# alibaba/loongcollector

Hardware: AMD Instinct MI355X
Metric: MB/s parsed (512B lines, 10-field regex) per MI355X + HBM-roofline % (higher is better)
Workload: dtype u8

## Files before the change

loongcollector_amd/csrc/gpu_runtime.hip:

```cpp
#include <hip/hip_runtime.h>

#include <type_traits>

#include <algorithm>
#include <atomic>
#include <cstdlib>
#include <map>
#include <mutex>
#include <cstdio>
#include <chrono>
#include <cstring>
#include <thread>
#include <string>
#include <vector>

#include "device_tables.h"
#include "grok_runtime.hpp"
#include "runtime_internal.hpp"
#include "nfa_kernel.hpp"
#include "nfa_wide_kernel.hpp"
#include "nfa_decide_kernel.hpp"
#include "bt_kernel.hpp"
#include "regex_handle.hpp"
#include "sched_kernel.hpp"
// ... 199 lines not shown

void lcReleaseDeviceTables(lc_regex* re) {
    int cur = 0;
    bool haveCur = hipGetDevice(&cur) == hipSuccess;
    {
        LcLazyTdfa& Z = re->lazy;
        for (int d = 0; d < kLcMaxDevices; ++d)
            if (Z.dBlob[d]) {
                Z.retired.emplace_back(d, Z.dBlob[d]);
                Z.dBlob[d] = nullptr;
            }
        for (const auto& r : Z.retired)
            if (hipSetDevice(r.first) == hipSuccess) (void)hipFree(r.second);
        Z.retired.clear();
    }
    for (int d = 0; d < kLcMaxDevices; ++d) {
        if (re->dTdfaBlob[d] || re->dNfaBlob[d] || re->dTdfaWideBlob[d] || re->dScreenBlob[d] || re->dTdfaL2Blob[d] || re->dBtBlob[d]) {
            if (hipSetDevice(d) == hipSuccess) {
                if (re->dBtBlob[d]) (void)hipFree(re->dBtBlob[d]);
                if (re->dTdfaL2Blob[d]) (void)hipFree(re->dTdfaL2Blob[d]);
                if (re->dScreenBlob[d]) (void)hipFree(re->dScreenBlob[d]);
                if (re->dTdfaBlob[d]) (void)hipFree(re->dTdfaBlob[d]);
                if (re->dTdfaWideBlob[d]) (void)hipFree(re->dTdfaWideBlob[d]);
                if (re->dNfaBlob[d]) (void)hipFree(re->dNfaBlob[d]);
            }
            re->dTdfaBlob[d] = re->dNfaBlob[d] = re->dTdfaWideBlob[d] = re->dScreenBlob[d] = re->dTdfaL2Blob[d] = re->dBtBlob[d] = nullptr;
        }
    }
    if (haveCur) (void)hipSetDevice(cur);
}

struct DoneRequest {
    uint32_t* counter = nullptr;
    uint32_t* flag = nullptr;
    uint32_t seq = 0;
    bool armed = false, consumed = false;
};
static thread_local DoneRequest tlsDone;
static thread_local bool tlsJobTableInPlace = false;

static int lcAllowLds(const void* kern, size_t lds) {
    if (lds <= 64 * 1024) return LC_OK;
    int dev = 0;
    HIP_TRY(hipGetDevice(&dev));
    static thread_local std::map<std::pair<const void*, int>, size_t> set;
    size_t& have = set[{kern, dev}];
    if (lds > have) {
        HIP_TRY(hipFuncSetAttribute(kern, hipFuncAttributeMaxDynamicSharedMemorySize, int(lds)));
        have = lds;
    }
    return LC_OK;
}

template <int BLOCK, bool PAIR, bool COMPACT = false>
static int launchTdfaBlock(const void* dBlob, uint32_t blobBytes, uint32_t regBytes, size_t lds, const uint8_t* d_data,
                           const uint32_t* d_off, const uint32_t* d_len, uint32_t sep, uint32_t minLen, uint32_t n, const uint32_t* d_n, const uint32_t* d_order, const uint32_t* d_resume, uint32_t ngroups,
                           int32_t* d_caps, uint8_t* d_status, hipStream_t stream, uint32_t* longFlag = nullptr, uint32_t seq = 0,
                           uint32_t nregsWord = 0, bool pairOne = false) {
    static const bool noGenOff = [] {
        const char* e = getenv("LC_TDFA_NOGEN");
        return e && e[0] == '0';
    }();
    const bool noGen = !PAIR && !noGenOff && (nregsWord & TD_NREGS_NO_GENERAL) != 0;
    constexpr bool kCanMopUp = BLOCK == 256 && !COMPACT;
    const bool mopUp = kCanMopUp && minLen != 0;
    constexpr int kMopUp = kCanMopUp ? kLabMopUp : 0;
    const void* kern;
    const char* name;
    if constexpr (PAIR) {
        constexpr int kOne = kTdfaNoGeneralPrograms | kLabPairOne | (COMPACT ? kLabDmaStage : 0);
        if (pairOne) {
            kern = mopUp ? reinterpret_cast<const void*>(tdfa_stream_kernel<BLOCK, COMPACT, true, kOne | kMopUp>)
                         : reinterpret_cast<const void*>(tdfa_stream_kernel<BLOCK, COMPACT, true, kOne>);
            name = COMPACT ? "tdfa_stream_kernel<compact,nogeneral,pair1,dma>" : "tdfa_stream_kernel<nogeneral,pair1>";
        } else {
            kern = mopUp ? reinterpret_cast<const void*>(tdfa_stream_kernel<BLOCK, COMPACT, true, kMopUp>)
                         : reinterpret_cast<const void*>(tdfa_stream_kernel<BLOCK, COMPACT, true>);
            name = COMPACT ? "tdfa_stream_kernel<compact,pair>" : "tdfa_stream_kernel<pair>";
        }
    } else if constexpr (COMPACT) {
        kern = noGen ? reinterpret_cast<const void*>(tdfa_stream_kernel<BLOCK, true, false, kTdfaNoGeneralPrograms | kLabDmaStage>)
                     : reinterpret_cast<const void*>(tdfa_stream_kernel<BLOCK, true, false, kLabDmaStage>);
        name = noGen ? "tdfa_stream_kernel<compact,nogeneral,dma>" : "tdfa_stream_kernel<compact,dma>";
    } else {
        if (noGen) kern = mopUp ? reinterpret_cast<const void*>(tdfa_stream_kernel<BLOCK, false, false, kTdfaNoGeneralPrograms | kMopUp>)
                                : reinterpret_cast<const void*>(tdfa_stream_kernel<BLOCK, false, false, kTdfaNoGeneralPrograms>);
        else kern = mopUp ? reinterpret_cast<const void*>(tdfa_stream_kernel<BLOCK, false, false, kMopUp>)
                          : reinterpret_cast<const void*>(tdfa_stream_kernel<BLOCK, false, false>);
        name = noGen ? "tdfa_stream_kernel<nogeneral>" : "tdfa_stream_kernel";
    }
    static const size_t extraLds = [] {
        const char* e = getenv("LC_TDFA_EXTRA_LDS");
        return e ? size_t(atol(e)) : size_t(0);
    }();
    lds += extraLds;
    if (const int rc = lcAllowLds(kern, lds); rc != LC_OK) return rc;
    uint32_t grid = (n + BLOCK - 1) / BLOCK;
    if (mopUp) grid = std::min(grid, 256u);
    noteKernel(name);
    const uint32_t* blobArg = static_cast<const uint32_t*>(dBlob);
    uint32_t* doneCounter = nullptr;
    uint32_t* doneFlag = nullptr;
    uint32_t doneSeq = 0;
    if (tlsDone.armed && minLen == 0 && longFlag == nullptr) {
        doneCounter = tlsDone.counter;
        doneFlag = tlsDone.flag;
        doneSeq = tlsDone.seq;
        tlsDone.consumed = true;
    }
    void* args[] = {&d_data, &d_off, &d_len, &sep, &minLen, &n, &d_n, &d_order, &d_resume, &blobArg, &blobBytes, &regBytes, &ngroups,
                    &d_caps, &d_status, &longFlag, &seq, &doneCounter, &doneFlag, &doneSeq};
    HIP_TRY(hipLaunchKernel(kern, dim3(grid), dim3(BLOCK), args, lds, stream));
    return LC_OK;
}

static bool lcPairOneFormat(const std::vector<uint32_t>& blob) {
    const uint32_t po = blob[TD_OFF_PAIR];
    return po != 0 && po / 4 + TP_FORMAT < blob.size() && blob[po / 4 + TP_FORMAT] == 1;
}

static int launchTdfa(lc_regex* re, int dev, const uint8_t* d_data, const uint32_t* d_off, const uint32_t* d_len,
                      uint32_t sep, uint32_t n, const uint32_t* d_n, const uint32_t* d_order, const uint32_t* d_resume, uint32_t ngroups, int32_t* d_caps,
                      uint8_t* d_status, hipStream_t stream);
static int launchTdfaL2Family(lc_regex* re, const uint32_t* hostBlob, const void* dBlob, bool waveByChoice, int dev, const uint8_t* d_data,
                              const uint32_t* d_off, const uint32_t* d_len, uint32_t sep, uint32_t n, const uint32_t* d_n,
                              const uint32_t* d_order, const uint32_t* d_resume, uint32_t ngroups, int32_t* d_caps, uint8_t* d_status,
                              hipStream_t stream, uint32_t* pendingFlag, uint32_t seq) {
// ... 1597 lines not shown
```

loongcollector_amd/csrc/tdfa_kernel.hpp:

```cpp
#pragma once

#include <hip/hip_runtime.h>

#include <type_traits>

#include "../../include/lc_regex_gpu.h"
#include "device_tables.h"

#ifndef LC_TDFA_MIN_WAVES
#define LC_TDFA_MIN_WAVES 1
#endif

typedef uint32_t u32x4 __attribute__((ext_vector_type(4)));
typedef uint32_t __attribute__((address_space(3))) * LdsWordPtr;
typedef u32x4 __attribute__((address_space(3))) * LdsQuadPtr;
typedef const uint8_t __attribute__((address_space(3))) * LdsBytePtr;
typedef const u32x4 __attribute__((address_space(1))) * GlobalQuadPtr;

template <typename RegT>
using LdsRegPtrT = RegT __attribute__((address_space(3))) *;
constexpr uint32_t kTdfaWideMaxLine = 0xFFFFu;

#ifndef LC_TDFA_STAGE_BYTES
#define LC_TDFA_STAGE_BYTES 64
#endif
constexpr uint32_t kTdfaStageBytes = LC_TDFA_STAGE_BYTES;
constexpr int kTdfaLoads = int(kTdfaStageBytes / 16);
constexpr uint32_t kTdfaRowStride = kTdfaStageBytes + 16;
constexpr uint32_t kTdfaStagePerWave = 64 * kTdfaRowStride;

__device__ __forceinline__ void tdfaWaveLdsSync() {
    __builtin_amdgcn_fence(__ATOMIC_ACQ_REL, "wavefront");
    __builtin_amdgcn_wave_barrier();
}

enum { kLabNoStamp = 1, kLabPreClass = 2, kLabGlobalClass = 4, kLabReplicated = 8, kLabNoOutput = 16, kLabNoLoop = 32, kLabNoGeneral = 64,
       kLabOneStamp = 128 ,
       kLabDmaStage = 256 ,
       kLabWaves5 = 512 ,
       kLabNoDmaWait = 1024 ,
       kLabPairOne = 4096 ,
       kLabMopUp = 8192  };
constexpr int kTdfaNoGeneralPrograms = kLabNoGeneral;

template <typename TdfaReg>
__device__ __forceinline__ uint32_t tdfaRegLane(uint32_t tid) {
    if constexpr (sizeof(TdfaReg) == 2) return (tid & ~63u) | ((tid & 31u) << 1) | ((tid >> 5) & 1u);
    else return tid;
}

template <int BLOCK, typename TdfaReg>
__device__ __forceinline__ void tdfaRunMoveList(uint8_t* smem, uint32_t regsBase, uint32_t list, uint32_t pos,
                                                uint32_t tid) {
    TdfaReg* regs = reinterpret_cast<TdfaReg*>(smem + regsBase);
    const uint32_t* hdr = reinterpret_cast<const uint32_t*>(smem);
    const uint32_t* opsStart = reinterpret_cast<const uint32_t*>(smem + hdr[TD_OFF_OPSSTART]);
    const uint16_t* ops = reinterpret_cast<const uint16_t*>(smem + hdr[TD_OFF_OPS]);
    const uint32_t at = opsStart[list];
    const uint32_t cnt = ops[at];
#pragma unroll 1
    for (uint32_t i = 0; i < cnt; ++i) {
        const uint32_t w = ops[at + 1 + i];
        const uint32_t dst = w & 0xFF, src = w >> 8;
        const TdfaReg val = (src == TD_REG_POS) ? TdfaReg(pos) : regs[src * BLOCK + tdfaRegLane<TdfaReg>(tid)];
        regs[dst * BLOCK + tdfaRegLane<TdfaReg>(tid)] = val;
    }
}

__device__ __forceinline__ uint32_t addLowHalf(uint32_t a, uint32_t t) {
    uint32_t r;
    asm("v_add_u32_sdwa %0, %1, %2 dst_sel:DWORD dst_unused:UNUSED_PAD src0_sel:DWORD src1_sel:WORD_0"
        : "=v"(r)
        : "v"(a), "v"(t));
    return r;
}
__device__ __forceinline__ uint32_t addHighHalf(uint32_t a, uint32_t t) {
    uint32_t r;
    asm("v_add_u32_sdwa %0, %1, %2 dst_sel:DWORD dst_unused:UNUSED_PAD src0_sel:DWORD src1_sel:WORD_1"
        : "=v"(r)
        : "v"(a), "v"(t));
    return r;
}

template <int BLOCK, typename TdfaReg, int LAB = 0>
__device__ __forceinline__ void tdfaReplayChunk(uint8_t* smem, u32x4 q, uint32_t t, uint32_t base, uint32_t L,
                                                uint32_t idCol, uint32_t regsBase, uint32_t tid, uint32_t nBytes) {
    typedef LdsRegPtrT<TdfaReg> LdsRegPtr;
    const LdsBytePtr cmap = reinterpret_cast<LdsBytePtr>(TD_CMAP_OFFSET);
    const uint32_t regAddr0 = regsBase + tdfaRegLane<TdfaReg>(tid) * sizeof(TdfaReg);
#pragma unroll 1
    for (uint32_t j = 0; j < nBytes; ++j) {
        const uint32_t word = (j < 8) ? ((j < 4) ? q.x : q.y) : ((j < 12) ? q.z : q.w);
        const uint32_t b = (word >> ((j & 3) * 8)) & 0xFFu;
        uint32_t col = (base + j < L) ? ((LAB & kLabPreClass) ? b : uint32_t(cmap[b])) : idCol;
        if constexpr ((LAB & kLabReplicated) != 0) col = (col << 4) + ((tid & 15u) << 2);
// ... 8 lines not shown
                                                   uint32_t regBytes) {
    if ((blob[TD_NREGS] >> 16) & 0x1FFFu) {
        uint32_t* regs = reinterpret_cast<uint32_t*>(smem + blobBytes);
        for (uint32_t i = threadIdx.x; i < regBytes / 4; i += BLOCK) regs[i] = 0;
    }
}

template <int BLOCK, typename TdfaReg, int LAB = 0>
__device__ __forceinline__ void tdfaWriteResults(uint8_t* smem, uint32_t tileAddr, uint32_t regsBase, uint32_t state, bool live,
                                                 uint32_t line, uint32_t L, uint32_t from, bool permuted, uint32_t nGroupsOut,
                                                 int32_t* __restrict__ caps, uint8_t* __restrict__ status) {
    const uint32_t* hdr = reinterpret_cast<const uint32_t*>(smem);
    const uint32_t tid = threadIdx.x, lane = tid & 63;
    const uint32_t nSlots = hdr[TD_NSLOTS];
    const uint16_t* finalId = reinterpret_cast<const uint16_t*>(smem + hdr[TD_OFF_FINALID]);
    const uint8_t* finalMap = smem + hdr[TD_OFF_FINALMAP];
    const TdfaReg* regs = reinterpret_cast<const TdfaReg*>(smem + regsBase);
    const uint32_t fid = live ? uint32_t(finalId[state]) : 0xFFFFu;
    const bool matched = live && (state != 0) && (fid != 0xFFFFu);
    const uint32_t nOut = 2 * nGroupsOut;
    const uint32_t rl = tdfaRegLane<TdfaReg>(tid);
    const uint32_t foldOff = ((hdr[TD_NREGS] >> 16) & 0x1FFFu) * 16;
    if (foldOff) {
        const uint32_t* fw = reinterpret_cast<const uint32_t*>(smem + foldOff);
        TdfaReg* rw = reinterpret_cast<TdfaReg*>(smem + regsBase) + tdfaRegLane<TdfaReg>(tid);
        const uint32_t nWords = __builtin_amdgcn_readfirstlane(fw[0]);
        for (uint32_t i0 = 0; i0 < nWords; i0 += 64) {
            const uint32_t fwv = (i0 + lane < nWords) ? fw[1 + i0 + lane] : 0xFFFFFF00u;
            const uint32_t cnt = nWords - i0 < 64 ? nWords - i0 : 64;
            for (uint32_t j0 = 0; j0 < cnt; j0 += 4) {
                uint32_t w[4];
                TdfaReg both[4];
#pragma unroll
                for (int k = 0; k < 4; ++k) {
                    w[k] = uint32_t(__builtin_amdgcn_readlane(int(fwv), int((j0 + k) & 63)));
                    both[k] = rw[(w[k] & 0xFFu) * BLOCK];
                }
#pragma unroll
                for (int k = 0; k < 4; ++k) {
                    if (j0 + k >= cnt) break;
                    if (!__any(both[k] != 0)) continue;
#pragma unroll
                    for (int m = 1; m < 4; ++m) {
                        const uint32_t r = (w[k] >> (8 * m)) & 0xFFu;
                        if (r != 0xFFu) {
                            const TdfaReg own = rw[r * BLOCK];
                            rw[r * BLOCK] = both[k] > own ? both[k] : own;
                        }
                    }
                }
            }
        }
    }
    if constexpr ((LAB & kLabPairOne) != 0) {
        const uint32_t* ph = reinterpret_cast<const uint32_t*>(smem + hdr[TD_OFF_PAIR]);
        const uint32_t dOff = ph[TP_OFF_DERIVE];
        if (dOff) {
            const uint32_t* dw = reinterpret_cast<const uint32_t*>(smem + dOff);
            TdfaReg* rw = reinterpret_cast<TdfaReg*>(smem + regsBase) + tdfaRegLane<TdfaReg>(tid);
            const uint32_t nWords = __builtin_amdgcn_readfirstlane(dw[0]);
            for (uint32_t i = 0; i < nWords; ++i) {
                const uint32_t w = __builtin_amdgcn_readfirstlane(dw[1 + i]);
                rw[(w & 0xFFu) * BLOCK] = TdfaReg(rw[((w >> 8) & 0xFFu) * BLOCK] + TdfaReg(w >> 16));
            }
        }
    }
    auto slotValue = [&](uint32_t s) -> int32_t {
        int32_t val = -1;
        if (matched && s < nSlots) {
            const uint32_t m = finalMap[fid * nSlots + s];
            if (m == TD_REG_POS) val = int32_t(L + from);
            else if (m != TD_REG_NONE) val = int32_t(regs[m * BLOCK + rl] + from);
        }
        return val;
    };
    constexpr uint32_t kTileWords = 1024;
    if (!permuted && nOut != 0 && nOut <= kTileWords && __all(live)) {
        int32_t* tile = reinterpret_cast<int32_t*>(smem + tileAddr);
        uint32_t rowsPerPass = kTileWords / nOut;
        if (rowsPerPass > 64) rowsPerPass = 64;
        if (rowsPerPass > 1) rowsPerPass &= ~1u;
        int32_t* gout = caps + size_t(line - lane) * nOut;
        const uint32_t fid0 = __builtin_amdgcn_readfirstlane(fid);
        const bool sameMap = __all(fid == fid0) && fid0 != 0xFFFFu;
        const int32_t end = int32_t(L + from);
        for (uint32_t p0 = 0; p0 < 64; p0 += rowsPerPass) {
            tdfaWaveLdsSync();
            const bool inPass = lane >= p0 && lane - p0 < rowsPerPass;
            int32_t* row = tile + (inPass ? lane - p0 : 0u) * nOut;
            if (sameMap) {
                const uint8_t* map = finalMap + fid0 * nSlots;
                for (uint32_t s0 = 0; s0 < nOut; s0 += 64) {
                    const uint32_t sl = s0 + lane;
                    const uint32_t mapv = (sl < nSlots && sl < nOut) ? uint32_t(map[sl]) : uint32_t(TD_REG_NONE);
                    const uint32_t cnt = nOut - s0 < 64 ? nOut - s0 : 64;
                    for (uint32_t k0 = 0; k0 < cnt; k0 += 8) {
                        int32_t v[8];
#pragma unroll
                        for (int k = 0; k < 8; ++k) {
                            const uint32_t m = uint32_t(__builtin_amdgcn_readlane(int(mapv), int((k0 + k) & 63)));
                            const uint32_t r = m < TD_REG_NONE ? m : 0u;
                            const int32_t reg = int32_t(regs[r * BLOCK + rl] + from);
                            int32_t val = m == TD_REG_POS ? end : reg;
                            val = m == TD_REG_NONE ? -1 : val;
                            v[k] = state != 0 ? val : -1;
                        }
                        if (inPass) {
#pragma unroll
                            for (int k = 0; k < 8; ++k)
                                if (k0 + k < cnt) row[s0 + k0 + k] = v[k];
                        }
                    }
                }
            } else if (inPass) {
#pragma unroll 4
                for (uint32_t s = 0; s < nOut; ++s) row[s] = slotValue(s);
            }
            tdfaWaveLdsSync();
            const uint32_t rows = 64 - p0 < rowsPerPass ? 64 - p0 : rowsPerPass;
            const uint32_t total = rows * nOut;
            int32_t* g = gout + size_t(p0) * nOut;
            if ((reinterpret_cast<uintptr_t>(g) & 15u) == 0 && (total & 3u) == 0) {
                typedef int32_t i32x4 __attribute__((ext_vector_type(4)));
                const uint32_t nq = total / 4;
                i32x4 q[4];
#pragma unroll
                for (int i = 0; i < 4; ++i) {
                    const uint32_t at = lane + 64u * uint32_t(i);
                    if (at < nq) q[i] = *reinterpret_cast<const i32x4 __attribute__((address_space(3)))*>(tileAddr + at * 16u);
                }
#pragma unroll
                for (int i = 0; i < 4; ++i) {
                    const uint32_t at = lane + 64u * uint32_t(i);
                    if (at < nq) __builtin_nontemporal_store(q[i], reinterpret_cast<i32x4*>(g) + at);
                }
            } else {
                for (uint32_t d = lane; d < total; d += 64) g[d] = tile[d];
            }
        }
    } else if (live) {
        int32_t* out = caps + size_t(line) * nOut;
        for (uint32_t s = 0; s < nOut; ++s) out[s] = slotValue(s);
    }
// ... 21 lines not shown
```

loongcollector_amd/csrc/tdfa_stream_kernel.hpp:

```cpp
#pragma once

#include "tdfa_kernel.hpp"

#ifndef LC_TDFA_STREAM_CHUNK
#define LC_TDFA_STREAM_CHUNK 8
#endif
#ifndef LC_TDFA_GCLASS
#define LC_TDFA_GCLASS 0
#endif
#ifndef LC_TDFA_STAMP_ISA
#define LC_TDFA_STAMP_ISA 1
#endif
#ifndef LC_TDFA_ROW_ALIGN
#define LC_TDFA_ROW_ALIGN 1
#endif
#ifndef LC_TDFA_STREAM_WAVES
#define LC_TDFA_STREAM_WAVES 4
#endif

constexpr uint32_t kTdfaIdColByteAddr = TD_ID_COL * 4;

template <int NB, bool CHECKED, typename TdfaReg, int LAB>
__device__ __forceinline__ uint32_t tdfaStreamChunk(uint32_t t, const uint32_t (&col)[NB], uint32_t (&ncol)[NB],
                                                    const uint32_t (&nwords)[NB / 4], uint32_t nbase, uint32_t L, uint32_t idCol,
// ... 24 lines not shown
#ifndef LC_TDFA_STREAM_NO_SCHED_BARRIER
        __builtin_amdgcn_sched_barrier(0);
#endif
    }
    seenOut = seen | t;
    return t;
}

template <int BLOCK, int NB, bool CHECKED, typename TdfaReg, int LAB = 0>
__device__ __forceinline__ uint32_t tdfaStreamPairChunk(uint32_t t, const uint32_t (&colp)[NB / 2], uint32_t (&na)[NB / 2],
                                                        uint32_t (&nc)[NB / 2], const uint32_t (&nwords)[NB / 4], uint32_t nbase,
                                                        uint32_t L, uint32_t cmapA, uint32_t idAAddr,
                                                        const uint32_t (&ptt)[NB / 2], uint32_t (&tt)[NB / 2], uint32_t pbase,
                                                        uint32_t regAddr0, uint32_t& seenOut) {
    typedef LdsRegPtrT<TdfaReg> LdsRegPtr;
    constexpr uint32_t kRegShift = (BLOCK == 1024 ? 12 : BLOCK == 512 ? 11 : BLOCK == 256 ? 10 : BLOCK == 128 ? 9 : 8) -
                                   (sizeof(TdfaReg) == 2 ? 1 : 0);
    uint32_t seen = 0;
    uint32_t pos = pbase;
#pragma unroll
    for (int p = 0; p < NB / 2; ++p) {
        t = *reinterpret_cast<LdsWordPtr>(addLowHalf(colp[p], t));
        tt[p] = t;
        uint32_t b0, b1;
        asm volatile("v_bfe_u32 %0, %1, %2, 8" : "=v"(b0) : "v"(nwords[p >> 1]), "n"((p & 1) * 16));
        asm volatile("v_bfe_u32 %0, %1, %2, 8" : "=v"(b1) : "v"(nwords[p >> 1]), "n"((p & 1) * 16 + 8));
        if constexpr (CHECKED) {
            na[p] = *reinterpret_cast<LdsHalfPtr>((nbase + 2 * p < L) ? cmapA + b0 * 2 : idAAddr);
            nc[p] = *reinterpret_cast<LdsBytePtr>((nbase + 2 * p + 1 < L) ? TD_CMAP_OFFSET + b1 : kTdfaIdColByteAddr);
        } else {
            na[p] = *reinterpret_cast<LdsHalfPtr>(cmapA + b0 * 2);
            nc[p] = *reinterpret_cast<LdsBytePtr>(TD_CMAP_OFFSET + b1);
        }
        if constexpr ((LAB & kLabOneStamp) != 0) {
            *reinterpret_cast<LdsRegPtr>(regAddr0 + (((ptt[p] >> 16) & 0xFu) << kRegShift)) = TdfaReg(pos);
            asm volatile("v_add_u32 %0, 2, %0" : "+v"(pos));
        } else {
            const uint32_t r0 = (ptt[p] >> 16) & 0xFFu, r1 = ptt[p] >> 24;
            *reinterpret_cast<LdsRegPtr>(regAddr0 + (r0 << kRegShift)) = TdfaReg(pos);
            asm volatile("v_add_u32 %0, 1, %0" : "+v"(pos));
            *reinterpret_cast<LdsRegPtr>(regAddr0 + (r1 << kRegShift)) = TdfaReg(pos);
            asm volatile("v_add_u32 %0, 1, %0" : "+v"(pos));
        }
        if constexpr ((LAB & kLabNoGeneral) == 0)
            if (p > 0) seen |= tt[p - 1];
#ifndef LC_TDFA_STREAM_NO_SCHED_BARRIER
        __builtin_amdgcn_sched_barrier(0);
#endif
    }
    seenOut = seen | t;
    return t;
}

template <int BLOCK, int NB, bool CHECKED, typename TdfaReg>
__device__ __forceinline__ uint32_t tdfaStreamPair1Chunk(uint32_t t, const uint32_t (&colp)[NB / 2], uint32_t (&na)[NB / 2],
                                                         uint32_t (&nc)[NB / 2], const uint32_t (&nwords)[NB / 4], uint32_t nbase,
                                                         uint32_t L, uint32_t cmapA, uint32_t idAAddr,
                                                         const uint32_t (&ptt)[NB / 2], uint32_t (&tt)[NB / 2], uint32_t pbase,
                                                         uint32_t regAddr0, const uint8_t* __restrict__ gcmap8 = nullptr) {
    typedef LdsRegPtrT<TdfaReg> LdsRegPtr;
    constexpr uint32_t kRegShift = (BLOCK == 1024 ? 12 : BLOCK == 512 ? 11 : BLOCK == 256 ? 10 : BLOCK == 128 ? 9 : 8) -
                                   (sizeof(TdfaReg) == 2 ? 1 : 0);
#pragma unroll
    for (int p = 0; p < NB / 2; ++p) {
        t = *reinterpret_cast<LdsWordPtr>(addLowHalf(colp[p], t));
        tt[p] = t;
        uint32_t b0, b1;
        asm volatile("v_bfe_u32 %0, %1, %2, 8" : "=v"(b0) : "v"(nwords[p >> 1]), "n"((p & 1) * 16));
        asm volatile("v_bfe_u32 %0, %1, %2, 8" : "=v"(b1) : "v"(nwords[p >> 1]), "n"((p & 1) * 16 + 8));
        if constexpr (CHECKED) {
            na[p] = *reinterpret_cast<LdsHalfPtr>((nbase + 2 * p < L) ? cmapA + b0 * 2 : idAAddr);
            nc[p] = *reinterpret_cast<LdsBytePtr>((nbase + 2 * p + 1 < L) ? TD_CMAP_OFFSET + b1 : kTdfaIdColByteAddr);
        } else {
            na[p] = *reinterpret_cast<LdsHalfPtr>(cmapA + b0 * 2);
#if LC_TDFA_GCLASS
            nc[p] = gcmap8[b1];
#else
            nc[p] = *reinterpret_cast<LdsBytePtr>(TD_CMAP_OFFSET + b1);
#endif
        }
#if LC_TDFA_STAMP_ISA
        if constexpr (LC_TDFA_ROW_ALIGN == 1) {
            uint32_t ra, delta, addr, val;
            asm("v_bfe_u32 %0, %1, 16, 7" : "=v"(ra) : "v"(ptt[p]));
            asm("v_lshl_add_u32 %0, %1, %2, %3" : "=v"(addr) : "v"(ra), "n"(kRegShift), "v"(regAddr0));
            asm("v_bfe_u32 %0, %1, 23, 1" : "=v"(delta) : "v"(ptt[p]));
            const uint32_t posU = __builtin_amdgcn_readfirstlane(pbase) + uint32_t(2 * p);
            asm("v_add_u32 %0, %1, %2" : "=v"(val) : "s"(posU), "v"(delta));
            *reinterpret_cast<LdsRegPtr>(addr) = TdfaReg(val);
        } else
#endif
        {
            const uint32_t ra = (ptt[p] >> 16) & 0x7Fu;
            *reinterpret_cast<LdsRegPtr>(regAddr0 + (ra << kRegShift)) = TdfaReg(pbase + uint32_t(2 * p) + ((ptt[p] >> 23) & 1u));
        }
#ifndef LC_TDFA_STREAM_NO_SCHED_BARRIER
        __builtin_amdgcn_sched_barrier(0);
#endif
    }
    return t;
}
template <int BLOCK, int NP, typename TdfaReg>
__device__ __forceinline__ void tdfaSettleDoubles(const uint32_t (&ptt)[NP], uint32_t pbase, uint32_t regAddr0) {
    typedef LdsRegPtrT<TdfaReg> LdsRegPtr;
    constexpr uint32_t kRegShift = (BLOCK == 1024 ? 12 : BLOCK == 512 ? 11 : BLOCK == 256 ? 10 : BLOCK == 128 ? 9 : 8) -
                                   (sizeof(TdfaReg) == 2 ? 1 : 0);
    uint32_t any = 0;
#pragma unroll
    for (int p = 0; p < NP; ++p) any |= ptt[p];
    if (!__any(int32_t(any) < 0)) return;
#pragma unroll
    for (int p = 0; p < NP; ++p) {
        if (int32_t(ptt[p]) < 0) {
            const LdsRegPtr reg = reinterpret_cast<LdsRegPtr>(regAddr0 + (((ptt[p] >> 24) & 0x7Fu) << kRegShift));
            const TdfaReg val = TdfaReg(pbase + uint32_t(2 * p) + 1u);
            const TdfaReg cur = *reg;
            *reg = cur > val ? cur : val;
        }
    }
}

__device__ __forceinline__ void tdfaDmaLoad16(uint32_t ldsDst, uint64_t base, uint32_t off) {
    uint32_t keep;
    asm volatile("s_mov_b32 %0, m0\n\ts_mov_b32 m0, %2\n\ts_nop 0\n\tglobal_load_lds_dwordx4 %1, %3\n\ts_mov_b32 m0, %0"
                 : "=&s"(keep)
                 : "v"(off), "s"(ldsDst), "s"(base)
                 : "memory");
}
__device__ __forceinline__ void tdfaDmaWait() { asm volatile("s_waitcnt vmcnt(0)" ::: "memory"); }
__device__ __forceinline__ void tdfaLdsDrain() { asm volatile("s_waitcnt lgkmcnt(0)" ::: "memory"); }

template <int BLOCK, bool COMPACT, bool PAIR, int LAB>
__device__ __forceinline__ void tdfaStreamBody(
    const uint8_t* __restrict__ data, const uint32_t* __restrict__ off, const uint32_t* __restrict__ len, uint32_t sepBytes,
    uint32_t minLen, uint32_t nLines, const uint32_t* __restrict__ nLinesPtr, const uint32_t* __restrict__ order,
    const uint32_t* __restrict__ resume, const uint32_t* __restrict__ blob, uint32_t blobBytes, uint32_t regBytes,
    uint32_t nGroupsOut, int32_t* __restrict__ caps, uint8_t* __restrict__ status, uint32_t* __restrict__ longFlag,
    uint32_t launchSeq, uint32_t blockId) {
    static_assert(kTdfaStageBytes == 64 || kTdfaStageBytes == 128, "4 or 8 16-byte segments per stage");
    constexpr int kLoads = kTdfaLoads;
    static_assert(!PAIR || (LAB & kLabPreClass) == 0, "no pre-classified pairs");
    typedef typename std::conditional<COMPACT, uint16_t, uint32_t>::type TdfaReg;
    typedef LdsRegPtrT<TdfaReg> LdsRegPtr;
    constexpr uint32_t kRowStride = COMPACT ? kTdfaStageBytes : kTdfaRowStride;
    constexpr uint32_t kStagePerWave = 64 * kRowStride;
    constexpr bool DMA = COMPACT && (LAB & kLabDmaStage) != 0 && kTdfaStageBytes == 64;
    constexpr bool PAIR1 = PAIR && (LAB & kLabPairOne) != 0;
    static_assert(!PAIR1 || (LAB & kLabNoGeneral) != 0, "one-stamp pair tables have no general register programs");
    extern __shared__ __attribute__((aligned(16))) uint8_t smem[];
    const uint32_t tid = threadIdx.x;
    if (nLinesPtr) {
        const uint32_t dyn = *nLinesPtr;
        nLines = dyn < nLines ? dyn : nLines;
    }
    if (minLen && longFlag && __atomic_load_n(longFlag, __ATOMIC_RELAXED) < launchSeq) return;
    if (minLen) {
        const uint32_t s0 = blockId * BLOCK + tid;
        bool mine = false;
        if (s0 < nLines) {
            const uint32_t ln = order ? order[s0] : s0;
            uint32_t l0 = len ? len[ln] : off[ln + 1] - off[ln] - sepBytes;
            if (resume) {
                const uint32_t f0 = resume[ln];
                l0 -= f0 < l0 ? f0 : l0;
            }
            mine = l0 >= minLen;
        }
        volatile uint32_t* flag = reinterpret_cast<volatile uint32_t*>(smem);
        if (tid == 0) *flag = 0;
        __syncthreads();
        if (mine) *flag = 1;
        __syncthreads();
        const bool any = *flag != 0;
        __syncthreads();
        if (!any) return;
    }
    {
        const uint4* src = reinterpret_cast<const uint4*>(blob);
        uint4* dst = reinterpret_cast<uint4*>(smem);
        for (uint32_t i = tid; i < blobBytes / 16; i += BLOCK) dst[i] = src[i];
        tdfaClearRegisters<BLOCK>(smem, blob, blobBytes, regBytes);
        if constexpr (PAIR1) {
            if (((blob[TD_NREGS] >> 16) & 0x1FFFu) == 0) {
                uint32_t* regs = reinterpret_cast<uint32_t*>(smem + blobBytes);
                for (uint32_t i = threadIdx.x; i < regBytes / 4; i += BLOCK) regs[i] = 0;
            }
        }
    }
    __syncthreads();
    const uint32_t* hdr = reinterpret_cast<const uint32_t*>(smem);
    const uint32_t rowBytes = hdr[TD_ROW_BYTES];
    const uint32_t idCol = hdr[TD_ID_COL];
    const uint32_t regsBase = blobBytes;
    const uint32_t dummyT = PAIR1 ? ((hdr[TD_NREGS] & 0xFFFFu) - 1) << 16 : PAIR ? ((hdr[TD_NREGS] & 0xFFFFu) - 1) * 0x01010000u : (((hdr[TD_NREGS] & 0xFFFFu) - 1) * BLOCK * uint32_t(sizeof(TdfaReg))) << 16;
    uint32_t t = hdr[TD_START_ROW];
    TdfaPairInfo pi{};
    uint32_t idAAddr = 0;
    auto walkRow = [&](uint32_t singleRow) {
        return PAIR ? pi.base + ((singleRow & 0xFFFFu) - TD_TRANS_OFFSET) / rowBytes * pi.rowBytes : singleRow;
    };
    if constexpr (PAIR) {
// ... 81 lines not shown
    u32x4 in[kLoads];
    u32x4 W[kLoads];
    if constexpr (DMA) {
        dmaStage(0);
        tdfaDmaWait();
#pragma unroll
        for (int k = 0; k < kLoads; ++k) W[k] = *reinterpret_cast<LdsQuadPtr>(myRow + ((uint32_t(k) * 16) ^ mySwizzle));
    } else {
#pragma unroll
        for (int i = 0; i < kLoads; ++i) {
            in[i] = u32x4{0, 0, 0, 0};
            if (seg < srcSpan[i]) in[i] = *reinterpret_cast<GlobalQuadPtr>(dataAligned + srcOff[i]);
        }
        tdfaWaveLdsSync();
#pragma unroll
        for (int i = 0; i < kLoads; ++i) *reinterpret_cast<LdsQuadPtr>(dstAddr[i]) = in[i];
        tdfaWaveLdsSync();
#pragma unroll
        for (int i = 0; i < kLoads; ++i) {
            in[i] = u32x4{0, 0, 0, 0};
            if (kTdfaStageBytes + seg < srcSpan[i]) in[i] = *reinterpret_cast<GlobalQuadPtr>(dataAligned + (srcOff[i] + kTdfaStageBytes));
        }
#pragma unroll
        for (int k = 0; k < kLoads; ++k) W[k] = *reinterpret_cast<LdsQuadPtr>(myRow + ((uint32_t(k) * 16) ^ mySwizzle));
    }
    constexpr int NB = LC_TDFA_STREAM_CHUNK;
    constexpr int kChunksPerStage = int(kTdfaStageBytes) / NB;
    auto rowWord = [&](int w) -> uint32_t {
        const u32x4& q = W[(w >> 2) & (kLoads - 1)];
        return (w & 3) == 0 ? q.x : (w & 3) == 1 ? q.y : (w & 3) == 2 ? q.z : q.w;
    };
    constexpr int NC = PAIR ? NB / 2 : NB;
    uint32_t col[NC], ptt[NC];
    {
        const uint32_t base0 = 0u - head;
#pragma unroll
        for (int j = 0; j < NB; ++j) {
            const uint32_t b = (rowWord(j >> 2) >> ((j & 3) * 8)) & 0xFFu;
            uint32_t c;
            if constexpr ((LAB & kLabPreClass) != 0) c = (base0 + j < L) ? b : idCol;
            else if (PAIR && (j & 1) == 0) c = *reinterpret_cast<LdsHalfPtr>((base0 + j < L) ? pi.cmapA + b * 2 : idAAddr);
            else c = *reinterpret_cast<LdsBytePtr>((base0 + j < L) ? TD_CMAP_OFFSET + b : kTdfaIdColByteAddr);
            if constexpr (PAIR) {
                if ((j & 1) == 0) col[j / 2] = c;
                else col[j / 2] += c;
            } else {
                col[j] = c;
            }
        }
#pragma unroll
        for (int j = 0; j < NC; ++j) ptt[j] = dummyT;
    }
    uint32_t pbase = 0;

    if constexpr ((LAB & kLabNoLoop) != 0) maxStages = 0;
    for (uint32_t s = 0; s < maxStages; ++s) {
        if constexpr (DMA) {
            tdfaLdsDrain();
            dmaStage((s + 1) * kTdfaStageBytes);
        } else {
            tdfaWaveLdsSync();
#pragma unroll
            for (int i = 0; i < kLoads; ++i) *reinterpret_cast<LdsQuadPtr>(dstAddr[i]) = in[i];
            tdfaWaveLdsSync();
            const uint32_t nextOff = (s + 2) * kTdfaStageBytes;
#pragma unroll
            for (int i = 0; i < kLoads; ++i) {
                in[i] = u32x4{0, 0, 0, 0};
                if (nextOff + seg < srcSpan[i]) in[i] = *reinterpret_cast<GlobalQuadPtr>(dataAligned + (srcOff[i] + nextOff));
            }
        }
        auto runChunks = [&](auto allFullTag, auto c0Tag, auto c1Tag) -> bool {
        constexpr bool ALLFULL = decltype(allFullTag)::value;
        constexpr int C0 = decltype(c0Tag)::value, C1 = decltype(c1Tag)::value;
#pragma unroll
        for (int c = C0; c < C1; ++c) {
            const uint32_t base = s * kTdfaStageBytes + uint32_t(c) * NB - head;
            if constexpr (!ALLFULL && PAIR1) {
                if (c > 0 && __all(s * kTdfaStageBytes + uint32_t(c) * NB >= head + L)) return true;
            }
            const uint32_t nbase = base + NB;
            const bool waveFull = PAIR1 && waveMaxHead <= s * kTdfaStageBytes + uint32_t(c + 1) * NB &&
                                  waveMinSpan >= s * kTdfaStageBytes + uint32_t(c + 2) * NB;
            const bool fullNext = ALLFULL || waveFull || (nbase < L && L - nbase >= uint32_t(NB));
            const uint32_t entry = t;
            uint32_t nwords[NB / 4], cwords[4] = {0, 0, 0, 0};
#pragma unroll
            for (int w = 0; w < NB / 4; ++w) {
                nwords[w] = rowWord(((c + 1) * NB / 4 + w) & (kLoads * 4 - 1));
                cwords[w] = rowWord(c * NB / 4 + w);
            }
            uint32_t ncol[NC], tt[NC], seen;
            bool general;
            if constexpr (PAIR1) {
                uint32_t na[NC], nc[NC];
                if (ALLFULL || waveFull || __all(fullNext)) t = tdfaStreamPair1Chunk<BLOCK, NB, false, TdfaReg>(t, col, na, nc, nwords, nbase, L, pi.cmapA, idAAddr, ptt, tt, pbase, regAddr0, reinterpret_cast<const uint8_t*>(blob) + TD_CMAP_OFFSET);
                else t = tdfaStreamPair1Chunk<BLOCK, NB, true, TdfaReg>(t, col, na, nc, nwords, nbase, L, pi.cmapA, idAAddr, ptt, tt, pbase, regAddr0);
                tdfaSettleDoubles<BLOCK, NC, TdfaReg>(ptt, pbase, regAddr0);
#pragma unroll
                for (int j = 0; j < NC; ++j) ncol[j] = na[j] + nc[j];
                seen = 0;
                general = false;
            } else if constexpr (PAIR) {
                uint32_t na[NC], nc[NC];
                if (__all(fullNext)) t = tdfaStreamPairChunk<BLOCK, NB, false, TdfaReg, LAB>(t, col, na, nc, nwords, nbase, L, pi.cmapA, idAAddr, ptt, tt, pbase, regAddr0, seen);
                else t = tdfaStreamPairChunk<BLOCK, NB, true, TdfaReg, LAB>(t, col, na, nc, nwords, nbase, L, pi.cmapA, idAAddr, ptt, tt, pbase, regAddr0, seen);
#pragma unroll
                for (int j = 0; j < NC; ++j) ncol[j] = na[j] + nc[j];
                general = (LAB & kLabNoGeneral) ? false : (seen & ((TP_GENERAL << 16) | (TP_GENERAL << 24))) != 0;
            } else {
                if (__all(fullNext)) t = tdfaStreamChunk<NB, false, TdfaReg, LAB>(t, col, ncol, nwords, nbase, L, idCol, ptt, tt, pbase, regAddr0, seen);
                else t = tdfaStreamChunk<NB, true, TdfaReg, LAB>(t, col, ncol, nwords, nbase, L, idCol, ptt, tt, pbase, regAddr0, seen);
                general = (LAB & kLabNoGeneral) ? false : (seen & (TD_OP_GENERAL << 16)) != 0;
            }
            if (__any(general)) {
                const u32x4 q = {cwords[0], cwords[1], cwords[2], cwords[3]};
                uint32_t single = entry;
                if constexpr (PAIR) single = TD_TRANS_OFFSET + ((entry & 0xFFFFu) - pi.base) / pi.rowBytes * rowBytes;
                tdfaReplayChunk<BLOCK, TdfaReg, LAB>(smem, q, single, base, L, idCol, regsBase, tid, NB);
#pragma unroll
                for (int j = 0; j < NC; ++j) tt[j] = dummyT;
            }
            if constexpr (DMA) {
                if (c == kChunksPerStage - 2) {
                    if constexpr ((LAB & kLabNoDmaWait) == 0) tdfaDmaWait();
#pragma unroll
                    for (int k = 0; k < kLoads - 1; ++k) W[k] = *reinterpret_cast<LdsQuadPtr>(myRow + ((uint32_t(k) * 16) ^ mySwizzle));
                } else if (c == kChunksPerStage - 1) {
                    W[kLoads - 1] = *reinterpret_cast<LdsQuadPtr>(myRow + ((uint32_t(kLoads - 1) * 16) ^ mySwizzle));
                }
            } else if ((c + 1) * NB % 16 == 0) {
                const int k = ((c + 1) * NB / 16 - 1) & (kLoads - 1);
                W[k] = *reinterpret_cast<LdsQuadPtr>(myRow + ((uint32_t(k) * 16) ^ mySwizzle));
            }
#pragma unroll
            for (int j = 0; j < NC; ++j) {
                col[j] = ncol[j];
                ptt[j] = tt[j];
            }
            pbase = base;
        }
        return false;
        };
        {
            using std::integral_constant;
            constexpr integral_constant<int, 0> k0{};
            constexpr integral_constant<int, 2> k2{};
            constexpr integral_constant<int, kChunksPerStage - 1> kLast{};
            constexpr integral_constant<int, kChunksPerStage> kEnd{};
            const uint32_t s0 = s * kTdfaStageBytes;
            const bool headsPastChunk0 = PAIR1 && waveMaxHead <= s0 + uint32_t(NB);
            const bool headsPastChunk2 = PAIR1 && waveMaxHead <= s0 + 3u * uint32_t(NB);
            const bool allNextInside = PAIR1 && waveMinSpan >= s0 + kTdfaStageBytes + uint32_t(NB);
            const bool nextInsideButLast = PAIR1 && waveMinSpan >= s0 + kTdfaStageBytes;
            if (headsPastChunk0 && allNextInside) {
                (void)runChunks(std::true_type{}, k0, kEnd);
            } else if (kChunksPerStage == 8 && headsPastChunk2 && allNextInside) {
                if (!runChunks(std::false_type{}, k0, k2)) (void)runChunks(std::true_type{}, k2, kEnd);
            } else if (kChunksPerStage == 8 && headsPastChunk0 && nextInsideButLast) {
                (void)runChunks(std::true_type{}, k0, kLast);
                (void)runChunks(std::false_type{}, kLast, kEnd);
            } else {
                (void)runChunks(std::false_type{}, k0, kEnd);
            }
        }
        if (__all((t & 0xFFFFu) == deadRow || s + 1 >= myStages)) break;
    }
    if constexpr (DMA) tdfaDmaWait();
    if constexpr (PAIR1) {
        constexpr uint32_t kRegShift = (BLOCK == 1024 ? 12 : BLOCK == 512 ? 11 : BLOCK == 256 ? 10 : BLOCK == 128 ? 9 : 8) -
                                       (sizeof(TdfaReg) == 2 ? 1 : 0);
#pragma unroll
        for (int j = 0; j < NC; ++j)
            *reinterpret_cast<LdsRegPtr>(regAddr0 + (((ptt[j] >> 16) & 0x7Fu) << kRegShift)) = TdfaReg(pbase + 2 * j + ((ptt[j] >> 23) & 1u));
        tdfaSettleDoubles<BLOCK, NC, TdfaReg>(ptt, pbase, regAddr0);
    } else if constexpr ((LAB & kLabNoStamp) == 0) {
        if constexpr (PAIR) {
            constexpr uint32_t kRegShift = (BLOCK == 1024 ? 12 : BLOCK == 512 ? 11 : BLOCK == 256 ? 10 : BLOCK == 128 ? 9 : 8) -
                                           (sizeof(TdfaReg) == 2 ? 1 : 0);
#pragma unroll
            for (int j = 0; j < NC; ++j) {
                *reinterpret_cast<LdsRegPtr>(regAddr0 + (((ptt[j] >> 16) & 0xFFu) << kRegShift)) = TdfaReg(pbase + 2 * j);
                *reinterpret_cast<LdsRegPtr>(regAddr0 + ((ptt[j] >> 24) << kRegShift)) = TdfaReg(pbase + 2 * j + 1);
            }
        } else {
#pragma unroll
            for (int j = 0; j < NC; ++j)
                *reinterpret_cast<LdsRegPtr>(addHighHalf(regAddr0, ptt[j])) = TdfaReg(pbase + j);
        }
    }

    if constexpr ((LAB & kLabNoOutput) != 0) {
        if (live && t == 0x12345u) status[line] = 3;
        return;
    }
    const uint32_t state = PAIR ? ((t & 0xFFFFu) - pi.base) / pi.rowBytes : ((t & 0xFFFFu) - TD_TRANS_OFFSET) / rowBytes;
    tdfaWriteResults<BLOCK, TdfaReg, LAB>(smem, stageBase, regsBase, state, live, line, L, from, order != nullptr, nGroupsOut, caps,
                                     status);
    };
    walkBlock(blockId);
}

template <int BLOCK, bool COMPACT, bool PAIR = false, int LAB = 0>
__global__ __launch_bounds__(BLOCK, (LAB & kLabWaves5) ? 5 : LC_TDFA_STREAM_WAVES) void tdfa_stream_kernel(
    const uint8_t* __restrict__ data, const uint32_t* __restrict__ off, const uint32_t* __restrict__ len, uint32_t sepBytes,
    uint32_t minLen, uint32_t nLines, const uint32_t* __restrict__ nLinesPtr, const uint32_t* __restrict__ order,
    const uint32_t* __restrict__ resume, const uint32_t* __restrict__ blob, uint32_t blobBytes, uint32_t regBytes,
    uint32_t nGroupsOut, int32_t* __restrict__ caps, uint8_t* __restrict__ status, uint32_t* __restrict__ longFlag,
    uint32_t launchSeq, uint32_t* __restrict__ doneCounter, uint32_t* __restrict__ doneFlag, uint32_t doneSeq) {
    if constexpr (!COMPACT && (LAB & kLabMopUp) != 0) {
        if (minLen) {
            if (longFlag && __atomic_load_n(longFlag, __ATOMIC_RELAXED) < launchSeq) return;
            const uint32_t nBlocks = (nLines + BLOCK - 1) / BLOCK;
            for (uint32_t b = blockIdx.x; b < nBlocks; b += gridDim.x) {
                tdfaStreamBody<BLOCK, COMPACT, PAIR, LAB>(data, off, len, sepBytes, minLen, nLines, nLinesPtr, order, resume, blob, blobBytes,
                                                         regBytes, nGroupsOut, caps, status, longFlag, launchSeq, b);
                __syncthreads();
            }
            tdfaSignalDone(doneCounter, doneFlag, doneSeq);
            return;
        }
    }
    tdfaStreamBody<BLOCK, COMPACT, PAIR, LAB>(data, off, len, sepBytes, minLen, nLines, nLinesPtr, order, resume, blob, blobBytes,
                                             regBytes, nGroupsOut, caps, status, longFlag, launchSeq, blockIdx.x);
    tdfaSignalDone(doneCounter, doneFlag, doneSeq);
}

struct TdfaJob {
// ... 21 lines not shown
```

Measured before the change: 3.193 million.

## Add deferred tag-register stamps and in-register derive for pair1 TDFA output

Adds a kLabDeferStamps kernel variant that buffers per-lane register-stamp events in two registers and flushes them to LDS only when a wave has a real pending event, instead of writing a stamp for every pair position. Separately, the output path computes derived register values in VGPRs via readlane chains when the row is small and the wave shares one final map, avoiding per-lane LDS derive writes. The deferred variant is gated by an env var defaulting to off, so only the row-in-registers output path is active by default. The trade-off is extra ALU and wave-vote work in the stream loop against fewer LDS stores.

```diff
diff --git a/loongcollector_amd/csrc/gpu_runtime.hip b/loongcollector_amd/csrc/gpu_runtime.hip
--- a/loongcollector_amd/csrc/gpu_runtime.hip
+++ b/loongcollector_amd/csrc/gpu_runtime.hip
@@ -275,6 +275,9 @@
     return LC_OK;
 }
 
+#ifndef LC_TDFA_DEFER_STAMPS_DEFAULT
+#define LC_TDFA_DEFER_STAMPS_DEFAULT 0
+#endif
 template <int BLOCK, bool PAIR, bool COMPACT = false>
 static int launchTdfaBlock(const void* dBlob, uint32_t blobBytes, uint32_t regBytes, size_t lds, const uint8_t* d_data,
                            const uint32_t* d_off, const uint32_t* d_len, uint32_t sep, uint32_t minLen, uint32_t n, const uint32_t* d_n, const uint32_t* d_order, const uint32_t* d_resume, uint32_t ngroups,
@@ -296,6 +299,14 @@
             kern = mopUp ? reinterpret_cast<const void*>(tdfa_stream_kernel<BLOCK, COMPACT, true, kOne | kMopUp>)
                          : reinterpret_cast<const void*>(tdfa_stream_kernel<BLOCK, COMPACT, true, kOne>);
             name = COMPACT ? "tdfa_stream_kernel<compact,nogeneral,pair1,dma>" : "tdfa_stream_kernel<nogeneral,pair1>";
+            if constexpr (COMPACT && LC_TDFA_ROW_ALIGN == 1) {
+                const char* e = getenv("LC_TDFA_DEFER_STAMPS");
+                const bool defer = e ? e[0] != '0' : bool(LC_TDFA_DEFER_STAMPS_DEFAULT);
+                if (defer) {
+                    kern = reinterpret_cast<const void*>(tdfa_stream_kernel<BLOCK, COMPACT, true, kOne | kLabDeferStamps>);
+                    name = "tdfa_stream_kernel<compact,nogeneral,pair1,dma,defer>";
+                }
+            }
         } else {
             kern = mopUp ? reinterpret_cast<const void*>(tdfa_stream_kernel<BLOCK, COMPACT, true, kMopUp>)
                          : reinterpret_cast<const void*>(tdfa_stream_kernel<BLOCK, COMPACT, true>);
diff --git a/loongcollector_amd/csrc/tdfa_kernel.hpp b/loongcollector_amd/csrc/tdfa_kernel.hpp
--- a/loongcollector_amd/csrc/tdfa_kernel.hpp
+++ b/loongcollector_amd/csrc/tdfa_kernel.hpp
@@ -40,7 +40,8 @@
        kLabWaves5 = 512 ,
        kLabNoDmaWait = 1024 ,
        kLabPairOne = 4096 ,
-       kLabMopUp = 8192  };
+       kLabMopUp = 8192 ,
+       kLabDeferStamps = 16384  };
 constexpr int kTdfaNoGeneralPrograms = kLabNoGeneral;
 
 template <typename TdfaReg>
@@ -155,17 +156,27 @@
             }
         }
     }
+    constexpr uint32_t kTileWords = 1024;
+    const bool viaTile = !permuted && nOut != 0 && nOut <= kTileWords && __all(live);
+    const uint32_t fid0 = __builtin_amdgcn_readfirstlane(fid);
+    const bool sameMap = __all(fid == fid0) && fid0 != 0xFFFFu;
+    constexpr uint32_t kRowRegs = 24;
+    uint32_t nDerive = 0;
+    const uint32_t* deriveWords = nullptr;
     if constexpr ((LAB & kLabPairOne) != 0) {
         const uint32_t* ph = reinterpret_cast<const uint32_t*>(smem + hdr[TD_OFF_PAIR]);
         const uint32_t dOff = ph[TP_OFF_DERIVE];
         if (dOff) {
-            const uint32_t* dw = reinterpret_cast<const uint32_t*>(smem + dOff);
-            TdfaReg* rw = reinterpret_cast<TdfaReg*>(smem + regsBase) + tdfaRegLane<TdfaReg>(tid);
-            const uint32_t nWords = __builtin_amdgcn_readfirstlane(dw[0]);
-            for (uint32_t i = 0; i < nWords; ++i) {
-                const uint32_t w = __builtin_amdgcn_readfirstlane(dw[1 + i]);
-                rw[(w & 0xFFu) * BLOCK] = TdfaReg(rw[((w >> 8) & 0xFFu) * BLOCK] + TdfaReg(w >> 16));
-            }
+            deriveWords = reinterpret_cast<const uint32_t*>(smem + dOff) + 1;
+            nDerive = __builtin_amdgcn_readfirstlane(deriveWords[-1]);
+        }
+    }
+    const bool rowInRegs = viaTile && sameMap && nOut <= kRowRegs && nDerive <= 64;
+    if (!rowInRegs && nDerive != 0) {
+        TdfaReg* rw = reinterpret_cast<TdfaReg*>(smem + regsBase) + tdfaRegLane<TdfaReg>(tid);
+        for (uint32_t i = 0; i < nDerive; ++i) {
+            const uint32_t w = __builtin_amdgcn_readfirstlane(deriveWords[i]);
+            rw[(w & 0xFFu) * BLOCK] = TdfaReg(rw[((w >> 8) & 0xFFu) * BLOCK] + TdfaReg(w >> 16));
         }
     }
     auto slotValue = [&](uint32_t s) -> int32_t {
@@ -177,21 +188,56 @@
         }
         return val;
     };
-    constexpr uint32_t kTileWords = 1024;
-    if (!permuted && nOut != 0 && nOut <= kTileWords && __all(live)) {
+    if (viaTile) {
         int32_t* tile = reinterpret_cast<int32_t*>(smem + tileAddr);
         uint32_t rowsPerPass = kTileWords / nOut;
         if (rowsPerPass > 64) rowsPerPass = 64;
         if (rowsPerPass > 1) rowsPerPass &= ~1u;
         int32_t* gout = caps + size_t(line - lane) * nOut;
-        const uint32_t fid0 = __builtin_amdgcn_readfirstlane(fid);
-        const bool sameMap = __all(fid == fid0) && fid0 != 0xFFFFu;
         const int32_t end = int32_t(L + from);
+        int32_t rowv[kRowRegs];
+        if (rowInRegs) {
+            const uint8_t* map = finalMap + fid0 * nSlots;
+            const uint32_t mapv = (lane < nSlots && lane < nOut) ? uint32_t(map[lane]) : uint32_t(TD_REG_NONE);
+            const uint32_t dwv = lane < nDerive ? deriveWords[lane] : 0u;
+            uint32_t root = mapv, dsum = 0;
+            for (uint32_t i = nDerive; i-- > 0;) {
+                const uint32_t w = uint32_t(__builtin_amdgcn_readlane(int(dwv), int(i)));
+                const bool hit = root == (w & 0xFFu);
+                root = hit ? (w >> 8) & 0xFFu : root;
+                dsum += hit ? w >> 16 : 0u;
+            }
+#pragma unroll
+            for (int k = 0; k < int(kRowRegs); k += 2) {
+                if (uint32_t(k) < nOut) {
+#pragma unroll
+                    for (int h = 0; h < 2; ++h) {
+                        const uint32_t m = uint32_t(__builtin_amdgcn_readlane(int(root), k + h));
+                        const uint32_t d = uint32_t(__builtin_amdgcn_readlane(int(dsum), k + h));
+                        const uint32_t r = m < TD_REG_NONE ? m : 0u;
+                        const int32_t reg = int32_t(TdfaReg(regs[r * BLOCK + rl] + TdfaReg(d)) + from);
+                        int32_t val = m == TD_REG_POS ? end : reg;
+                        val = m == TD_REG_NONE ? -1 : val;
+                        rowv[k + h] = state != 0 ? val : -1;
+                    }
+                }
+            }
+        }
         for (uint32_t p0 = 0; p0 < 64; p0 += rowsPerPass) {
             tdfaWaveLdsSync();
             const bool inPass = lane >= p0 && lane - p0 < rowsPerPass;
             int32_t* row = tile + (inPass ? lane - p0 : 0u) * nOut;
-            if (sameMap) {
+            if (rowInRegs) {
+                if (inPass) {
+#pragma unroll
+                    for (int k = 0; k < int(kRowRegs); k += 2) {
+                        if (uint32_t(k) < nOut) {
+                            row[k] = rowv[k];
+                            row[k + 1] = rowv[k + 1];
+                        }
+                    }
+                }
+            } else if (sameMap) {
                 const uint8_t* map = finalMap + fid0 * nSlots;
                 for (uint32_t s0 = 0; s0 < nOut; s0 += 64) {
                     const uint32_t sl = s0 + lane;
diff --git a/loongcollector_amd/csrc/tdfa_stream_kernel.hpp b/loongcollector_amd/csrc/tdfa_stream_kernel.hpp
--- a/loongcollector_amd/csrc/tdfa_stream_kernel.hpp
+++ b/loongcollector_amd/csrc/tdfa_stream_kernel.hpp
@@ -100,12 +100,44 @@
     return t;
 }
 
-template <int BLOCK, int NB, bool CHECKED, typename TdfaReg>
+__device__ __forceinline__ uint32_t tdfaDeferEvent(uint32_t entry, uint32_t posU) {
+    return (entry & 0x00FF0000u) | posU;
+}
+template <int BLOCK, typename TdfaReg>
+__device__ __forceinline__ void tdfaDeferStore(uint32_t ev, uint32_t regAddr0) {
+    typedef LdsRegPtrT<TdfaReg> LdsRegPtr;
+    constexpr uint32_t kRegShift = (BLOCK == 1024 ? 12 : BLOCK == 512 ? 11 : BLOCK == 256 ? 10 : BLOCK == 128 ? 9 : 8) -
+                                   (sizeof(TdfaReg) == 2 ? 1 : 0);
+    uint32_t ra, delta, addr;
+    asm("v_bfe_u32 %0, %1, 16, 7" : "=v"(ra) : "v"(ev));
+    asm("v_lshl_add_u32 %0, %1, %2, %3" : "=v"(addr) : "v"(ra), "n"(kRegShift), "v"(regAddr0));
+    asm("v_bfe_u32 %0, %1, 23, 1" : "=v"(delta) : "v"(ev));
+    *reinterpret_cast<LdsRegPtr>(addr) = TdfaReg(ev + delta);
+}
+template <int BLOCK, typename TdfaReg>
+__device__ __forceinline__ void tdfaDeferFlush(uint32_t& e0, uint32_t& e1, uint32_t dummyEv, uint32_t regAddr0) {
+    tdfaDeferStore<BLOCK, TdfaReg>(e1, regAddr0);
+    tdfaDeferStore<BLOCK, TdfaReg>(e0, regAddr0);
+    e0 = dummyEv;
+    e1 = dummyEv;
+}
+template <int BLOCK, typename TdfaReg>
+__device__ __forceinline__ void tdfaDeferPush(uint32_t entry, uint32_t posU, uint32_t& e0, uint32_t& e1, uint32_t dummyEv,
+                                              uint32_t regAddr0) {
+    const uint32_t ev = tdfaDeferEvent(entry, posU);
+    const bool real = (entry & 0x007F0000u) != dummyEv;
+    e1 = real ? e0 : e1;
+    e0 = real ? ev : e0;
+    if (__any(e1 != dummyEv)) tdfaDeferFlush<BLOCK, TdfaReg>(e0, e1, dummyEv, regAddr0);
+}
+
+template <int BLOCK, int NB, bool CHECKED, typename TdfaReg, int LAB = 0>
 __device__ __forceinline__ uint32_t tdfaStreamPair1Chunk(uint32_t t, const uint32_t (&colp)[NB / 2], uint32_t (&na)[NB / 2],
                                                          uint32_t (&nc)[NB / 2], const uint32_t (&nwords)[NB / 4], uint32_t nbase,
                                                          uint32_t L, uint32_t cmapA, uint32_t idAAddr,
                                                          const uint32_t (&ptt)[NB / 2], uint32_t (&tt)[NB / 2], uint32_t pbase,
-                                                         uint32_t regAddr0, const uint8_t* __restrict__ gcmap8 = nullptr) {
+                                                         uint32_t regAddr0, uint32_t& e0, uint32_t& e1, uint32_t dummyEv,
+                                                         const uint8_t* __restrict__ gcmap8 = nullptr) {
     typedef LdsRegPtrT<TdfaReg> LdsRegPtr;
     constexpr uint32_t kRegShift = (BLOCK == 1024 ? 12 : BLOCK == 512 ? 11 : BLOCK == 256 ? 10 : BLOCK == 128 ? 9 : 8) -
                                    (sizeof(TdfaReg) == 2 ? 1 : 0);
@@ -127,6 +159,10 @@
             nc[p] = *reinterpret_cast<LdsBytePtr>(TD_CMAP_OFFSET + b1);
 #endif
         }
+        if constexpr ((LAB & kLabNoStamp) != 0) {
+        } else if constexpr ((LAB & kLabDeferStamps) != 0) {
+            tdfaDeferPush<BLOCK, TdfaReg>(ptt[p], __builtin_amdgcn_readfirstlane(pbase) + uint32_t(2 * p), e0, e1, dummyEv, regAddr0);
+        } else
 #if LC_TDFA_STAMP_ISA
         if constexpr (LC_TDFA_ROW_ALIGN == 1) {
             uint32_t ra, delta, addr, val;
@@ -148,8 +184,9 @@
     }
     return t;
 }
-template <int BLOCK, int NP, typename TdfaReg>
-__device__ __forceinline__ void tdfaSettleDoubles(const uint32_t (&ptt)[NP], uint32_t pbase, uint32_t regAddr0) {
+template <int BLOCK, int NP, typename TdfaReg, int LAB = 0>
+__device__ __forceinline__ void tdfaSettleDoubles(const uint32_t (&ptt)[NP], uint32_t pbase, uint32_t regAddr0, uint32_t& e0,
+                                                  uint32_t& e1, uint32_t dummyEv) {
     typedef LdsRegPtrT<TdfaReg> LdsRegPtr;
     constexpr uint32_t kRegShift = (BLOCK == 1024 ? 12 : BLOCK == 512 ? 11 : BLOCK == 256 ? 10 : BLOCK == 128 ? 9 : 8) -
                                    (sizeof(TdfaReg) == 2 ? 1 : 0);
@@ -157,6 +194,7 @@
 #pragma unroll
     for (int p = 0; p < NP; ++p) any |= ptt[p];
     if (!__any(int32_t(any) < 0)) return;
+    if constexpr ((LAB & kLabDeferStamps) != 0) tdfaDeferFlush<BLOCK, TdfaReg>(e0, e1, dummyEv, regAddr0);
 #pragma unroll
     for (int p = 0; p < NP; ++p) {
         if (int32_t(ptt[p]) < 0) {
@@ -195,6 +233,9 @@
     constexpr bool DMA = COMPACT && (LAB & kLabDmaStage) != 0 && kTdfaStageBytes == 64;
     constexpr bool PAIR1 = PAIR && (LAB & kLabPairOne) != 0;
     static_assert(!PAIR1 || (LAB & kLabNoGeneral) != 0, "one-stamp pair tables have no general register programs");
+    constexpr bool DEFER = PAIR1 && (LAB & kLabDeferStamps) != 0;
+    static_assert(!DEFER || (COMPACT && LC_TDFA_ROW_ALIGN == 1), "deferred stamps: 16-bit positions, wave-uniform pair positions");
+    constexpr int kStampLab = LAB & (kLabDeferStamps | kLabNoStamp);
     extern __shared__ __attribute__((aligned(16))) uint8_t smem[];
     const uint32_t tid = threadIdx.x;
     if (nLinesPtr) {
@@ -382,6 +423,8 @@
         for (int j = 0; j < NC; ++j) ptt[j] = dummyT;
     }
     uint32_t pbase = 0;
+    const uint32_t dummyEv = PAIR1 ? __builtin_amdgcn_readfirstlane(dummyT) : 0u;
+    uint32_t e0 = dummyEv, e1 = dummyEv;
 
     if constexpr ((LAB & kLabNoLoop) != 0) maxStages = 0;
     for (uint32_t s = 0; s < maxStages; ++s) {
@@ -424,9 +467,9 @@
             bool general;
             if constexpr (PAIR1) {
                 uint32_t na[NC], nc[NC];
-                if (ALLFULL || waveFull || __all(fullNext)) t = tdfaStreamPair1Chunk<BLOCK, NB, false, TdfaReg>(t, col, na, nc, nwords, nbase, L, pi.cmapA, idAAddr, ptt, tt, pbase, regAddr0, reinterpret_cast<const uint8_t*>(blob) + TD_CMAP_OFFSET);
-                else t = tdfaStreamPair1Chunk<BLOCK, NB, true, TdfaReg>(t, col, na, nc, nwords, nbase, L, pi.cmapA, idAAddr, ptt, tt, pbase, regAddr0);
-                tdfaSettleDoubles<BLOCK, NC, TdfaReg>(ptt, pbase, regAddr0);
+                if (ALLFULL || waveFull || __all(fullNext)) t = tdfaStreamPair1Chunk<BLOCK, NB, false, TdfaReg, kStampLab>(t, col, na, nc, nwords, nbase, L, pi.cmapA, idAAddr, ptt, tt, pbase, regAddr0, e0, e1, dummyEv, reinterpret_cast<const uint8_t*>(blob) + TD_CMAP_OFFSET);
+                else t = tdfaStreamPair1Chunk<BLOCK, NB, true, TdfaReg, kStampLab>(t, col, na, nc, nwords, nbase, L, pi.cmapA, idAAddr, ptt, tt, pbase, regAddr0, e0, e1, dummyEv);
+                if constexpr ((LAB & kLabNoStamp) == 0) tdfaSettleDoubles<BLOCK, NC, TdfaReg, kStampLab>(ptt, pbase, regAddr0, e0, e1, dummyEv);
 #pragma unroll
                 for (int j = 0; j < NC; ++j) ncol[j] = na[j] + nc[j];
                 seen = 0;
@@ -497,13 +540,20 @@
         if (__all((t & 0xFFFFu) == deadRow || s + 1 >= myStages)) break;
     }
     if constexpr (DMA) tdfaDmaWait();
-    if constexpr (PAIR1) {
+    if constexpr (PAIR1 && (LAB & kLabNoStamp) != 0) {
+    } else if constexpr (DEFER) {
+#pragma unroll
+        for (int j = 0; j < NC; ++j)
+            tdfaDeferPush<BLOCK, TdfaReg>(ptt[j], __builtin_amdgcn_readfirstlane(pbase) + uint32_t(2 * j), e0, e1, dummyEv, regAddr0);
+        tdfaDeferFlush<BLOCK, TdfaReg>(e0, e1, dummyEv, regAddr0);
+        tdfaSettleDoubles<BLOCK, NC, TdfaReg>(ptt, pbase, regAddr0, e0, e1, dummyEv);
+    } else if constexpr (PAIR1) {
         constexpr uint32_t kRegShift = (BLOCK == 1024 ? 12 : BLOCK == 512 ? 11 : BLOCK == 256 ? 10 : BLOCK == 128 ? 9 : 8) -
                                        (sizeof(TdfaReg) == 2 ? 1 : 0);
 #pragma unroll
         for (int j = 0; j < NC; ++j)
             *reinterpret_cast<LdsRegPtr>(regAddr0 + (((ptt[j] >> 16) & 0x7Fu) << kRegShift)) = TdfaReg(pbase + 2 * j + ((ptt[j] >> 23) & 1u));
-        tdfaSettleDoubles<BLOCK, NC, TdfaReg>(ptt, pbase, regAddr0);
+        tdfaSettleDoubles<BLOCK, NC, TdfaReg>(ptt, pbase, regAddr0, e0, e1, dummyEv);
     } else if constexpr ((LAB & kLabNoStamp) == 0) {
         if constexpr (PAIR) {
             constexpr uint32_t kRegShift = (BLOCK == 1024 ? 12 : BLOCK == 512 ? 11 : BLOCK == 256 ? 10 : BLOCK == 128 ? 9 : 8) -
```

New measurement: 3.232 million, median of 6. 1.01x the previous value.
